# AppleHolic/pytorch_sound

Hardware: AMD Instinct MI355X
Metric: audio-sec/s STFT+mel+fwd/bwd (higher is better)
Workload: dtype bf16; 1 GPU; configs[1]: Conv1d separator (4 x ResBlock1, C=256, on 513-bin magnitude), 22.05 kHz, STFT 1024/256, 80 mel, batch 32 x 2 s per GPU, Adam, bf16 autocast; global_batch=32, parallelism=dp1, model_params=5520386

## Files before the change

### include/psnd.h

```cpp
#ifndef PSND_H
#define PSND_H

#include <stdint.h>
#include <stddef.h>

#ifdef __cplusplus
extern "C" {
#endif

#define PSND_OK 0
#define PSND_E_ARG (-1)
#define PSND_E_SHAPE (-2)
#define PSND_E_HIP (-3)
#define PSND_E_UNSUPPORTED (-4)

#define PSND_FRAMING_CENTER 0
#define PSND_FRAMING_HIFIGAN 1
#define PSND_FRAMING_NONE 2

int psnd_version(void);
const char *psnd_last_error(void);
#ifdef PSND_LAB
void psnd_env_refresh(void);
#endif
// ... 41 lines not shown
                  float eps, void *scratch, size_t scratch_bytes, float *out, void *stream);

#define PSND_LOG_NONE 0
#define PSND_LOG_E 1
#define PSND_LOG_10 2
size_t psnd_mel_plan_bytes(int M, int K);
int psnd_mel_plan_build(int M, int K, const float *mel_filter_host, void *plan_host);
int psnd_mel_fwd(const float *mag, int64_t N, int64_t F, int M, int K, const void *mel_plan,
                 int log_kind, float log_offset, float pre_clamp_min, float clamp_lo, float clamp_hi,
                 float *out, float *mel_lin, void *stream);
int psnd_mel_bwd(const float *gout, const float *mel_lin, int64_t N, int64_t F, int M, int K,
                 const void *mel_plan, int log_kind, float log_offset, float pre_clamp_min,
                 float clamp_lo, float clamp_hi, float *gmag, void *stream);

int psnd_logmel_fwd(const float *wav, int64_t N, int64_t T, int n_fft, int hop, int framing, const void *stft_plan,
                    float mag_eps, int M, const void *mel_plan, int log_kind, float log_offset, float pre_clamp_min,
                    float clamp_lo, float clamp_hi, float *out, void *stream);

int psnd_conv1d_cl(const void *A, const void *A2, const void *AM, float a2_slope, const void *W, const float *bias,
                   const void *res, const void *mask_src, int64_t N, int Lp, int L, int HP, int Ca, int Cb, int k,
                   int off0, int dstep, float act_slope, float mask_slope, void *out_raw, void *out_act,
                   void *a_eff_out, void *stream);
int psnd_conv1d_cl_wgrad_splits(int64_t N, int Lp, int Ca, int Cb, int k);
int psnd_conv1d_cl_pair_supported(int C, int k, int off1, int dstep1, int off2, int dstep2);
int psnd_conv1d_cl_pair(const void *A, const void *W1, const float *bias1, const void *M1, float m1_slope, float act1_slope,
                        void *mid_out, const void *W2, const float *bias2, const void *M2, float m2_slope, const void *res,
                        int64_t N, int Lp, int L, int HP, int C, int k, int off1, int dstep1, int off2, int dstep2,
                        float act2_slope, void *out_raw, void *out_act, void *stream);
typedef struct psnd_wgrad_desc {
    const void *g, *xa;
    float *gw_part, *gbias_part;
    int off0, dstep;
    int Ca, Cb, k, splits;
} psnd_wgrad_desc;
int psnd_conv1d_cl_wgrad_multi_splits(int64_t N, int Lp, int Ca, int Cb, int k, int n_convs);
int psnd_conv1d_cl_wgrad_multi(const psnd_wgrad_desc *d, int n, int64_t N, int Lp, void *stream);
typedef struct psnd_chain_pair {
    const void *W1;
    const float *bias1;
    float act1_slope;
    void *mid_out;
    const void *W2;
    const float *bias2;
    int off1, dstep1, off2, dstep2;
    float act2_slope;
    void *out_raw, *out_act;
// ... 18 lines not shown
int psnd_mel_l1_fwd_nfk(const float *mag_nfk, int64_t N, int64_t F, int M, int K, const void *mel_plan, int log_kind, float log_offset,
                        float pre_clamp_min, float clamp_lo, float clamp_hi, const float *ref, float *mel_lin, double *part, void *stream);
int psnd_mel_l1_bwd_nfk(const float *ref, const float *mel_lin, const float *g, float coef, int64_t N, int64_t F, int M, int K,
                        const void *mel_plan, int log_kind, float log_offset, float pre_clamp_min, float clamp_lo, float clamp_hi,
                        float *gmag_nfk, void *stream);
int64_t psnd_mask_head_l1_blocks(int64_t N, int64_t T, int Cp);
int psnd_mask_head_l1_fwd(const void *y, const float *mag, const float *ref, int64_t N, int C, int64_t T, int Lp, int HP, int Cp,
                          float *est, double *part, void *stream);
int psnd_mask_head_l1_bwd(const float *gest, const float *mag, const void *y, const float *est, const float *ref, const float *g,
                          float coef, int64_t N, int C, int64_t T, int Lp, int HP, int Cp, void *gy, void *stream);
int64_t psnd_mel_l1_blocks(int64_t N, int64_t F, int M);
int psnd_mel_l1_fwd(const float *mag, int64_t N, int64_t F, int M, int K, const void *mel_plan, int log_kind, float log_offset,
                    float pre_clamp_min, float clamp_lo, float clamp_hi, const float *ref, float *mel_lin, double *part, void *stream);
int psnd_mel_l1_bwd(const float *ref, const float *mel_lin, const float *g, float coef, int64_t N, int64_t F, int M, int K,
                    const void *mel_plan, int log_kind, float log_offset, float pre_clamp_min, float clamp_lo, float clamp_hi,
                    float *gmag, void *stream);
int psnd_nan_flag(const float *x, int64_t n, float *flag, void *stream);
int psnd_l1_loss_combine(const double *const *parts, const int64_t *nb, const double *scale, int terms, float *out, float *nan_flag, void *stream);
int psnd_conv_stats(int64_t *out4, int reset);
int psnd_conv_pair_stats(int64_t *out4, int reset);
int psnd_conv1d_cl_wgrad(const void *G1, const void *G2, const void *GM, float g2_slope, const void *xa, int64_t N,
                         int Lp, int Ca, int Cb, int k, int off0, int dstep, float *gw_part, float *gbias_part,
                         void *g_out, void *stream);
int psnd_conv1d_prep(const float *v, const float *g, const float *bias, int Cout, int Cin, int k, int Cb, int Ca,
                     void *wf, void *wb, float *bias_padded, void *stream);
int psnd_convtr1d_prep(const float *v, const float *g, const float *bias, int Cin, int Cout, int K, int stride, int Cr, int Cip,
                       void *wf, void *wb, float *bias_rep, void *stream);
int psnd_convtr1d_prep_multi(const void *descs_dev, int n, int total_blocks, void *stream);
int psnd_convtr1d_cl_fwd(const void *xa, const void *wf, const float *bias_rep, int64_t N, int Lp, int L, int HP, int Cip, int Cr,
                         int stride, int padding, int LpO, int HPO, float act_slope, void *out_raw, void *out_act, void *stream);
int psnd_convtr1d_cl_wgrad_splits(int64_t N, int Lp, int Cip, int Cr, int stride);
int psnd_convtr1d_cl_bwd(const void *g_raw, const void *g_act, const void *act, float act_slope, const void *wb, const void *xa,
                         int64_t N, int Lp, int L, int HP, int Cip, int Cr, int stride, int padding, int LpO, int HPO, void *gx,
                         void *g_eff, float *gw_part, void *stream);
int psnd_convtr1d_wnorm_bwd(const float *gw_part, int splits, const float *v, const float *g, int Cin, int Cout, int K, int stride,
                            int Cr, int Cip, float *gv, float *gg, void *stream);
int psnd_cl_mean_act_fwd(const void *a, const void *b, const void *c, const void *d, int count, float slope, void *out, int64_t n,
                         void *stream);
int psnd_cl_mean_act_bwd(const void *g, const void *y, int count, float slope, void *gin, int64_t n, void *stream);
int psnd_cl_sum2(const void *const *a, int na, void *out_a, const void *const *b, int nb, void *out_b, int64_t n, void *stream);
int psnd_cl_colsum_splits(int64_t rows, int C);
int psnd_cl_colsum(const void *g, int64_t rows, int C, int Lp, int lo, int hi, float *part, float *out, void *stream);
int psnd_conv1d_prep_multi(const void *descs_dev, int n, int total_blocks, int max_row, int which, void *stream);
#define PSND_WNORM_MAX 32
typedef struct psnd_wnorm_desc {
    const float *gw_part, *gbias_part;
// ... 154 lines not shown
```

### pytorch_sound_amd/_lib.py

```python
import ctypes
import os
import numpy as np

_HERE = os.path.dirname(os.path.abspath(__file__))
LIB_PATH = os.environ.get('PSND_LIB', os.path.join(_HERE, 'libpsnd_hip.so'))

PSND_OK = 0
FRAMING_CENTER = 0
FRAMING_HIFIGAN = 1
FRAMING_NONE = 2
LOG_NONE, LOG_E, LOG_10 = 0, 1, 2

_c = ctypes
_P = _c.c_void_p
_I64 = _c.c_int64
_INT = _c.c_int
_F = _c.c_float
_D = _c.c_double
_U32 = _c.c_uint32
_U64 = _c.c_uint64

SIGNATURES = {
    'psnd_version': (_INT, []),
    'psnd_last_error': (_c.c_char_p, []),
# ... 3 lines not shown
    'psnd_stream_wait_event': (_INT, [_P, _P]),
    'psnd_event_external_supported': (_INT, []),
    'psnd_frame_count': (_I64, [_I64, _INT, _INT, _INT]),
    'psnd_frame_sample_index': (_I64, [_I64, _INT, _I64, _INT, _INT, _INT]),
    'psnd_stft_plan_bytes': (_c.c_size_t, [_INT]),
    'psnd_stft_plan_build': (_INT, [_INT, _P, _P]),
    'psnd_stft_fwd': (_INT, [_P, _I64, _I64, _INT, _INT, _INT, _P, _F, _P, _P, _P, _P, _P]),
    'psnd_stft_mag_nfk': (_INT, [_P, _I64, _I64, _INT, _INT, _INT, _P, _F, _P, _P]),
    'psnd_stft_bwd': (_INT, [_P, _I64, _I64, _INT, _INT, _INT, _P, _F, _P, _P, _P, _P, _P]),
    'psnd_istft': (_INT, [_P, _P, _I64, _I64, _INT, _INT, _P, _F, _P, _P]),
    'psnd_stft_mr_plan_bytes': (_c.c_size_t, [_INT]),
    'psnd_stft_mr_plan_build': (_INT, [_INT, _P, _P]),
    'psnd_stft_mr_fwd': (_INT, [_P, _I64, _I64, _INT, _INT, _INT, _P, _c.c_size_t, _F, _P, _P, _P, _P, _P]),
    'psnd_stft_mr_bwd_scratch_bytes': (_c.c_size_t, [_I64, _I64, _INT, _INT, _INT]),
    'psnd_stft_mr_bwd': (_INT, [_P, _I64, _I64, _INT, _INT, _INT, _P, _c.c_size_t, _F, _P, _P, _P, _P, _c.c_size_t, _P, _P]),
    'psnd_istft_mr_scratch_bytes': (_c.c_size_t, [_I64, _I64, _INT]),
    'psnd_istft_mr': (_INT, [_P, _P, _I64, _I64, _INT, _INT, _P, _c.c_size_t, _F, _P, _c.c_size_t, _P, _P]),
    'psnd_mel_plan_bytes': (_c.c_size_t, [_INT, _INT]),
    'psnd_mel_plan_build': (_INT, [_INT, _INT, _P, _P]),
    'psnd_mel_fwd': (_INT, [_P, _I64, _I64, _INT, _INT, _P, _INT, _F, _F, _F, _F, _P, _P, _P]),
    'psnd_mel_bwd': (_INT, [_P, _P, _I64, _I64, _INT, _INT, _P, _INT, _F, _F, _F, _F, _P, _P]),
    'psnd_logmel_fwd': (_INT, [_P, _I64, _I64, _INT, _INT, _INT, _P, _F, _INT, _P, _INT, _F, _F, _F, _F, _P, _P]),
    'psnd_conv1d_cl': (_INT, [_P, _P, _P, _F, _P, _P, _P, _P, _I64, _INT, _INT, _INT, _INT, _INT, _INT, _INT, _INT, _F, _F, _P, _P, _P, _P]),
    'psnd_conv1d_cl_pair_supported': (_INT, [_INT, _INT, _INT, _INT, _INT, _INT]),
    'psnd_conv1d_cl_pair': (_INT, [_P, _P, _P, _P, _F, _F, _P, _P, _P, _P, _F, _P, _I64, _INT, _INT, _INT, _INT, _INT, _INT, _INT, _INT, _INT, _F, _P, _P, _P]),
    'psnd_conv1d_cl_wgrad': (_INT, [_P, _P, _P, _F, _P, _I64, _INT, _INT, _INT, _INT, _INT, _INT, _P, _P, _P, _P]),
    'psnd_conv1d_prep': (_INT, [_P, _P, _P, _INT, _INT, _INT, _INT, _INT, _P, _P, _P, _P]),
    'psnd_conv1d_wnorm_bwd': (_INT, [_P, _P, _INT, _P, _P, _INT, _INT, _INT, _INT, _INT, _P, _P, _P, _P]),
    'psnd_conv1d_cl_bwd': (_INT, [_P, _P, _P, _F, _P, _P, _I64, _INT, _INT, _INT, _INT, _INT, _INT, _INT, _INT, _P, _P, _P, _F, _P, _P, _P, _P]),
    'psnd_conv1d_cl_wgrad_multi_splits': (_INT, [_I64, _INT, _INT, _INT, _INT, _INT]),
    'psnd_conv1d_cl_wgrad_multi': (_INT, [_P, _INT, _I64, _INT, _P]),
    'psnd_nan_flag': (_INT, [_P, _I64, _P, _P]),
    'psnd_conv1d_cl_chain_rows': (_INT, [_INT, _INT, _INT, _P]),
    'psnd_conv1d_cl_chain_plan': (_INT, [_INT, _INT, _INT, _P, _I64, _P]),
    'psnd_conv1d_cl_chain': (_INT, [_P, _P, _P, _INT, _I64, _INT, _INT, _INT, _INT, _INT, _P]),
    'psnd_conv_chain_stats': (None, [_P]),
    'psnd_conv1d_cl_pair_bwd_supported': (_INT, [_INT, _INT, _INT, _INT, _INT, _INT]),
    'psnd_conv1d_cl_pair_bwd_splits': (_INT, [_I64, _INT, _INT, _INT]),
    'psnd_conv1d_cl_pair_bwd': (_INT, [_P, _P, _P, _F, _P, _P, _P, _F, _P, _I64, _INT, _INT, _INT, _INT, _INT, _INT, _INT, _INT, _INT, _P, _P, _P, _P,
                                       _P, _P, _INT, _INT, _P, _P, _P]),
    'psnd_conv1d_wnorm_bwd_multi': (_INT, [_P, _INT, _P]),
    'psnd_conv1d_prep_multi': (_INT, [_P, _INT, _INT, _INT, _INT, _P]),
    'psnd_conv1d_cl_wgrad_splits': (_INT, [_I64, _INT, _INT, _INT, _INT]),
    'psnd_mask_head_l1_blocks': (_I64, [_I64, _I64, _INT]),
    'psnd_masked_l1_blocks': (_I64, [_I64]),
    'psnd_masked_l1_fwd': (_INT, [_P, _P, _P, _I64, _INT, _I64, _P, _P, _P, _P]),
# ... 238 lines not shown
```

### pytorch_sound_amd/cl.py

```python
import ctypes
from collections import namedtuple
from pytorch_sound_amd import _switches as _sw
import weakref

import torch

from . import _lib
from ._lib import lib, check, ptr, stream_ptr

ALIGN_C = 32


def round_up(x, m):
    return (x + m - 1) // m * m


class CLShape:

    def __init__(self, N, L, HP):
        self.N, self.L, self.HP = int(N), int(L), int(HP)
        self.Lp = round_up(self.L + 2 * self.HP, 8)

    @property
    def R(self):
# ... 398 lines not shown

def branch_streams(dev, n):
    pool = _BRANCH_STREAMS.setdefault(dev.index, [])
    while len(pool) < n:
        pool.append(torch.cuda.Stream(device=dev))
    return pool[:n]


_WGRAD_STREAMS = {}


def _wgrad_streams(dev):
    if _sw.lab('PSND_CL_BWD_SPLIT', '0') != '1' or not _pair_enabled() or not AUTO_SECTIONS:
        return []
    n = int(_sw.lab('PSND_CL_WGRAD_STREAMS', '3'))
    pool = _WGRAD_STREAMS.setdefault(dev.index, [])
    while len(pool) < n:
        pool.append(torch.cuda.Stream(device=dev))
    return pool[:n]


def _pair_enabled():
    return _sw.lab('PSND_CL_PAIR', '1') != '0'


_Step = namedtuple('_Step', 'Cout Cin k Ca Cb dil pad slope has_res has_bias role')
_Conv = namedtuple('_Conv', 'inp wf bp res Ca Cb k off0 dil oslope raw act')
_Pair = namedtuple('_Pair', 'inp1 wf1 bp1 slope1 mid wf2 bp2 res C k off1 dstep1 off2 dstep2 oslope raw act')
_Chain = namedtuple('_Chain', 'inp1 res C k pairs')
_B = namedtuple('_B', 'G1 G2 am slope wb inp Ca Cb k pad dil gx g_out ep_mask ep_slope ep_res gw gbp S')
_W = namedtuple('_W', 'G1 G2 am slope inp Ca Cb k off0 dil gw gbp S')
_Side = namedtuple('_Side', 'w')
_PairB = namedtuple('_PairB', 'G wb2 m1 m1s g_h wb1 m2 m2s res C k off1 dstep1 off2 dstep2 gx flush_after')
_ChainB = namedtuple('_ChainB', 'pairs')
_PB = namedtuple('_PB', 'G wb2 m1 m1s g_h wb1 m2 m2s C k pad2 dil2 pad1 dil1 gx gw gbp lag')
_PBFlush = namedtuple('_PBFlush', 'lag')
_Lag = namedtuple('_Lag', 'g xa off0 dstep gw gbp C k')
_WBatch = namedtuple('_WBatch', 'conv G inp off0 dstep')


def _chain_takes(pairs):
    taps = [t for p in pairs for t in (p.off1, p.dstep1, p.off2, p.dstep2)]
    return lib().psnd_conv1d_cl_chain_rows(pairs[0].C, pairs[0].k, len(pairs), (ctypes.c_int * len(taps))(*taps)) >= 32


def _chain_pairs_bwd(plan, rows):
# ... 416 lines not shown
            last = i == n - 1
            inp, slope, has_res = src, (last_act_slope if last else 0.1), role in ('c2', 'r2')
            mk = lambda: torch.empty((shape.N, shape.Lp, Cb), dtype=torch.bfloat16, device=dev)
            if role == 'c1':
                raw, act, res, oslope = None, mk(), None, slope
                pending = act
            elif role == 'tail':
                raw, act, res, oslope = mk(), None, None, 1.0
                cur_x, cur_xa = raw, None
            else:
                raw, act, res, oslope = (mk() if (not last) or want_raw else None), mk(), (cur_x if has_res else None), slope
                cur_x, cur_xa = raw, act
            c1 = plan[-1] if plan else None
            if (role == 'c2' and _pair_enabled() and isinstance(c1, _Conv) and steps[-1].role == 'c1' and c1.Ca == Ca == Cb
                    and c1.k == k and lib().psnd_conv1d_cl_pair_supported(Ca, k, c1.off0, c1.dil, -pad, dil)):
                plan[-1] = _Pair(c1.inp, c1.wf, c1.bp, c1.oslope, c1.act, wf, bp, res, Ca, k, c1.off0, c1.dil, -pad, dil, oslope, raw, act)
            else:
                plan.append(_Conv(inp, wf, bp, res, Ca, Cb, k, -pad, dil, oslope, raw, act))
            steps.append(_Step(Cout, Cin, k, Ca, Cb, dil, pad, slope, has_res, b is not None, role))
            saved += [inp, act if act is not None else inp, wb, v32, g32]
        nsec, sides = _sections(dev, shape.N, shape.N * shape.Lp)
        Nh = shape.N // nsec
        plan = _chain_pairs(plan, Nh * shape.Lp)

        def run(h):
            st = stream_ptr(dev)
            q = lambda t: ptr(_sec(t, h, nsec))
            for e in plan:
                if isinstance(e, _Chain):
                    inp1, res0, C, k, pairs = e
                    arr = (_lib.ChainPair * len(pairs))()
                    for d, p in zip(arr, pairs):
                        d.W1, d.bias1, d.act1_slope, d.mid_out = p.wf1.data_ptr(), p.bp1.data_ptr(), float(p.slope1), q(p.mid)
                        d.W2, d.bias2, d.off1, d.dstep1, d.off2, d.dstep2 = p.wf2.data_ptr(), p.bp2.data_ptr(), p.off1, p.dstep1, p.off2, p.dstep2
                        d.act2_slope, d.out_raw, d.out_act = float(p.oslope), (q(p.raw) if p is pairs[-1] else None), q(p.act)
                    check(lib().psnd_conv1d_cl_chain(q(inp1), q(res0), ctypes.addressof(arr), len(pairs), Nh, shape.Lp, shape.L, shape.HP,
                                                     C, k, st), 'psnd_conv1d_cl_chain')
                    continue
                if isinstance(e, _Pair):
                    inp1, wf1, bp1, slope1, mid, wf2, bp2, res, C, k, off1, dstep1, off2, dstep2, oslope, raw, act = e
                    check(lib().psnd_conv1d_cl_pair(q(inp1), ptr(wf1), ptr(bp1), None, 1.0, float(slope1), q(mid), ptr(wf2), ptr(bp2),
                                                    None, 1.0, q(res), Nh, shape.Lp, shape.L, shape.HP, C, k, off1, dstep1, off2, dstep2,
                                                    float(oslope), q(raw), q(act), st), 'psnd_conv1d_cl_pair')
                    continue
                inp, wf, bp, res, Ca, Cb, k, off0, dil, oslope, raw, act = e
                check(lib().psnd_conv1d_cl(q(inp), None, None, 1.0, ptr(wf), ptr(bp), q(res), None,
                                           Nh, shape.Lp, shape.L, shape.HP, Ca, Cb, k, off0, dil, float(oslope), 1.0,
                                           q(raw), q(act), None, st), 'psnd_conv1d_cl')

        with torch.cuda.device(dev):
            _run_sections(dev, nsec, sides, run)
        ctx.steps, ctx.shape = steps, shape
        ctx.param_refs = params
        note_param_use(ctx, *params)
        ctx.save_for_backward(*saved)
        return cur_x, cur_xa

    @staticmethod
    def backward(ctx, g_raw, g_act):
        saved, steps, shape = ctx.saved_tensors, ctx.steps, ctx.shape
        dev = saved[0].device
        n = len(steps)
        if ctx.pack_owner is not None:
            ctx.pack_owner.write_backward_packs()
        g_raw = None if g_raw is None else g_raw.contiguous()
        g_act = None if g_act is None else g_act.contiguous()
        grads = [None] * (3 * n)
        descs, keep = [None] * n, []
# ... 8 lines not shown
                pv, pg, pb = prefs[3 * i:3 * i + 3]
                gv, gg = sink.dest(pv, pv.numel()), sink.dest(pg, pg.numel())
                gb = sink.dest(pb, Cb) if pb is not None else None
                early[i] = [(0, pv) if gv is not None else None, (1, pg) if gg is not None else None,
                            (2, pb) if gb is not None else None]
            gv = torch.empty_like(v32) if gv is None else gv.view_as(v32)
            gg = torch.empty_like(g32) if gg is None else gg.view_as(g32)
            gb = torch.empty(Cb, dtype=torch.float32, device=dev) if gb is None else gb
            return gv, gg, gb

        nsec, sides = _sections(dev, shape.N, shape.N * shape.Lp)
        wstreams = _wgrad_streams(dev) if shape.N * shape.Lp <= 8192 else []
        if wstreams:
            nsec, sides = 1, []
        Nh = shape.N // nsec
        plan = []
        skip = -1
        batch = (nsec == 1 and not wstreams and _pair_enabled() and _sw.lab('PSND_CL_BWD_BATCH', '1') == '1'
                 and shape.N * shape.Lp <= 8192)
        wbatch = []
        own_launch = []
        pair_bwd = nsec == 1 and not wstreams and not batch and _pair_enabled() and shape.N * shape.Lp <= 8192
        lag = None
        with torch.cuda.device(dev):
            g_comb = None
            res_pending = None
            def slabs(i, G1, G2, am, inp, S=None):
                s = steps[i]
                v32, g32 = saved[5 * i + 3], saved[5 * i + 4]
                if S is None:
                    S = lib().psnd_conv1d_cl_wgrad_splits(Nh, shape.Lp, s.Ca, s.Cb, s.k)
                gw = torch.empty((nsec * S, s.k, s.Cb, s.Ca), dtype=torch.float32, device=dev)
                gbp = torch.empty((nsec * S, s.Cb), dtype=torch.float32, device=dev)
                gv, gg, gb = grad_out(i, v32, g32, s.Cb)
                descs[i] = _lib.WnormDesc(gw.data_ptr(), gbp.data_ptr(), v32.data_ptr(), g32.data_ptr(), gv.data_ptr(), gg.data_ptr(),
                                          gb.data_ptr(), nsec * S, s.Cout, s.Cin, s.k, s.Cb, s.Ca)
                keep.extend([gw, gbp, G1, G2])
                grads[3 * i], grads[3 * i + 1] = gv, gg
                grads[3 * i + 2] = gb[:s.Cout] if s.has_bias else None
                return _W(G1, G2, am, s.slope, inp, s.Ca, s.Cb, s.k, -s.pad, s.dil, gw, gbp, S)

            for i in range(n - 1, -1, -1):
                if i == skip:
                    continue
                Cout, Cin, k, Ca, Cb, dil, pad, slope, has_res, has_bias, role = steps[i]
                inp, act, wb = saved[5 * i:5 * i + 3]
# ... 15 lines not shown
                        wl = slabs(i - 1, g_h, None, None, inp1, S2)
                        lag = _Lag(g_h, inp1, -p.pad, p.dil, wl.gw, wl.gbp, Ca, k)
                    else:
                        if batch:
                            wbatch += [_WBatch(i, G, inp, -pad, dil), _WBatch(i - 1, g_h, inp1, -p.pad, p.dil)]
                        else:
                            plan.append(_Side(slabs(i, G, None, None, inp)))
                        plan.append(_PairB(G, wb, inp, m1s, g_h, wb1, inp1, m2s, G, Ca, k, pad, -dil, p.pad, -p.dil, gx, len(wbatch)))
                        if not batch:
                            plan.append(_Side(slabs(i - 1, g_h, None, None, inp1)))
                    keep.extend([g_h, gx])
                    res_pending = G
                    g_comb = gx
                    skip = i - 1
                    continue
                if g_comb is None:
                    if g_raw is None and g_act is None:
                        raise _lib.PsndError('CL conv chain backward: no incoming gradient')
                    G1, G2 = g_raw, g_act
                    am = act if g_act is not None else None
                    need_gout = has_res and g_act is not None
                else:
                    G1, G2, am, need_gout = g_comb, None, None, False
                w = slabs(i, G1, G2, am, inp)
                g_out = torch.empty((shape.N, shape.Lp, Cb), dtype=torch.bfloat16, device=dev) if need_gout else None
                keep.append(g_out)
                g_here = g_out if need_gout else G1
                if i == 0 and not (ctx.needs_input_grad[0] or ctx.needs_input_grad[1]):
                    gx = None
                    plan.append(_Side(w) if wstreams else w)
                else:
                    gx = torch.empty((shape.N, shape.Lp, Ca), dtype=torch.bfloat16, device=dev)
                    if i == 0:
                        ep_mask, ep_res = None, None
                    elif role == 'c1':
                        ep_mask, ep_res = inp, res_pending
                    elif role == 'r2':
                        ep_mask, ep_res = inp, g_here
                    else:
                        ep_mask, ep_res = inp, None
                    plan.append(_B(G1, G2, am, slope, wb, inp, Ca, Cb, k, pad, dil, gx, g_out, ep_mask,
                                   float(p.slope if i > 0 else 1.0), ep_res, w.gw, w.gbp, w.S))
                own_launch.append((plan[-1], i))
                if role == 'c2':
                    res_pending = g_here
                if i > 0:
                    g_comb = gx
# ... 40 lines not shown
                        check(lib().psnd_conv1d_cl_pair_bwd(None, None, None, 1.0, None, None, None, 1.0, None, shape.N, shape.Lp, shape.L,
                                                            shape.HP, lg.C, lg.k, 0, 1, 0, 1, None, None, None, None, ptr(lg.g), ptr(lg.xa),
                                                            lg.off0, lg.dstep, ptr(lg.gw), ptr(lg.gbp), st), 'psnd_conv1d_cl_pair_bwd')
                        continue
                    if isinstance(e, _ChainB):
                        arr = (_lib.ChainPair * len(e.pairs))()
                        for d, p in zip(arr, e.pairs):
                            d.W1, d.bias1, d.act1_slope, d.mid_out = p.wb2.data_ptr(), None, 1.0, p.g_h.data_ptr()
                            d.W2, d.bias2, d.off1, d.dstep1, d.off2, d.dstep2 = p.wb1.data_ptr(), None, p.off1, p.dstep1, p.off2, p.dstep2
                            d.act2_slope, d.out_raw, d.out_act = 1.0, p.gx.data_ptr(), None
                            d.M1, d.M2, d.m1_slope, d.m2_slope = p.m1.data_ptr(), p.m2.data_ptr(), p.m1s, p.m2s
                        p0 = e.pairs[0]
                        check(lib().psnd_conv1d_cl_chain(ptr(p0.G), ptr(p0.G), ctypes.addressof(arr), len(e.pairs), shape.N, shape.Lp, shape.L,
                                                         shape.HP, p0.C, p0.k, st), 'psnd_conv1d_cl_chain')
                        continue
                    if isinstance(e, _PairB):
                        G, wb2, m1, m1s, g_h, wb1, m2, m2s, res, C, k, off1, dstep1, off2, dstep2, gx, _ = e
                        check(lib().psnd_conv1d_cl_pair(ptr(G), ptr(wb2), None, ptr(m1), m1s, 1.0, ptr(g_h), ptr(wb1), None, ptr(m2), m2s,
                                                        ptr(res), shape.N, shape.Lp, shape.L, shape.HP, C, k, off1, dstep1, off2, dstep2, 1.0,
                                                        ptr(gx), None, st), 'psnd_conv1d_cl_pair')
                        continue
                    if isinstance(e, _W):
                        G1, G2, am, slope, inp, Ca, Cb, k, off0, dil, gw, gbp, S = e
                        check(lib().psnd_conv1d_cl_wgrad(q(G1), q(G2), q(am), float(slope), q(inp), Nh, shape.Lp, Ca, Cb, k, off0, dil,
                                                         ptr(gw[h * S:(h + 1) * S]), ptr(gbp[h * S:(h + 1) * S]), None, st),
                              'psnd_conv1d_cl_wgrad')
                    else:
                        G1, G2, am, slope, wb, inp, Ca, Cb, k, pad, dil, gx, g_out, ep_mask, ep_slope, ep_res, gw, gbp, S = e
                        check(lib().psnd_conv1d_cl_bwd(q(G1), q(G2), q(am), float(slope), ptr(wb), q(inp), Nh, shape.Lp, shape.L,
                                                       shape.HP, Ca, Cb, k, pad, dil, q(gx), q(g_out), q(ep_mask), ep_slope, q(ep_res),
                                                       ptr(gw[h * S:(h + 1) * S]), ptr(gbp[h * S:(h + 1) * S]), st),
                              'psnd_conv1d_cl_bwd')

            st = stream_ptr(dev)
            handed = set()

            def wgrad_batch(part):
                for j0 in range(0, len(part), 32):
                    sub = part[j0:j0 + 32]
                    shp = [(steps[b.conv].Ca, steps[b.conv].Cb, steps[b.conv].k) for b in sub]
                    Ca, Cb, k = max(set(shp), key=shp.count)
                    cnt = max(shp.count((Ca, Cb, k)), len(wbatch) // 2) if len(part) < len(wbatch) else shp.count((Ca, Cb, k))
                    Sb = lib().psnd_conv1d_cl_wgrad_multi_splits(shape.N, shape.Lp, Ca, Cb, k, cnt)
                    arr = (_lib.WgradDesc * len(sub))()
                    for d, b in zip(arr, sub):
                        w = slabs(b.conv, b.G, None, None, b.inp, Sb)
# ... 119 lines not shown
```

### pytorch_sound_amd/csrc/psnd_conv.hip

```cpp
#include "psnd_common.h"
#include "psnd_conv_pair.h"
#include <stdlib.h>
#include <string.h>
#include <algorithm>
#include <atomic>

namespace {

typedef __attribute__((ext_vector_type(8))) short bf16x8;
typedef __attribute__((ext_vector_type(16))) float f32x16;
typedef unsigned short bf16_t;

__device__ __forceinline__ float bf2f(bf16_t v) { return __builtin_bit_cast(float, (unsigned)v << 16); }
__device__ __forceinline__ bf16_t f2bf(float f) {
    unsigned u = __builtin_bit_cast(unsigned, f);
    if ((u & 0x7fffffffu) > 0x7f800000u) return (bf16_t)((u >> 16) | 0x40);
    u += 0x7fffu + ((u >> 16) & 1u);
    return (bf16_t)(u >> 16);
}

typedef __bf16 hwbf16x2 __attribute__((ext_vector_type(2)));
typedef float f32x2_t __attribute__((ext_vector_type(2)));
__device__ __forceinline__ unsigned pack_bf16(float lo, float hi) {
    const f32x2_t v = {lo, hi};
// ... 1712 lines not shown
    const int wk = narrow_w ? 4 * WKT : pair_wk(k <= 3 ? 3 : (k <= 7 ? 7 : (k <= 11 ? 11 : 16)), 25);
    const int tx = (Cb + 63) / 64, ty = (Ca + 63) / 64 * ((k + wk - 1) / wk);
    int64_t target = 192;
    if (narrow_w) {
        target = 192;
        if (const char *e = PSND_ENV("PSND_WGRAD_BLOCKS_NARROW")) target = psnd_env_int(e, target, 1, 65535);
    }
    if (const char *e = PSND_ENV("PSND_WGRAD_BLOCKS")) target = psnd_env_int(e, target, 1, 65535);
    int64_t splits = target / ((int64_t)tx * ty);
    if (splits < 1) splits = 1;
    int64_t rps = (R + splits - 1) / splits;
    rps = (rps + 31) / 32 * 32;
    if (rps < 64) rps = 64;
    splits = (R + rps - 1) / rps;
    if (rps_out) *rps_out = rps;
    return (int)splits;
}

extern "C" int psnd_conv1d_cl_wgrad_splits(int64_t N, int Lp, int Ca, int Cb, int k) {
    if (N <= 0 || Lp <= 0 || Ca <= 0 || Cb <= 0 || k <= 0) return 0;
    return wgrad_splits(N * (int64_t)Lp, Ca, Cb, k, nullptr);
}

extern "C" int psnd_conv1d_cl_wgrad(const void *G1, const void *G2, const void *GM, float g2_slope, const void *xa, int64_t N,
                                    int Lp, int Ca, int Cb, int k, int off0, int dstep, float *gw_part, float *gbias_part,
                                    void *g_out, void *stream) {
    if ((!G1 && !G2) || (G2 && !GM) || !xa || !gw_part) PSND_FAIL(PSND_E_ARG, "conv1d_cl_wgrad: null pointer");
    if (Ca % 8 != 0 || Cb % 8 != 0 || k < 1 || k > 16 || N < 0) PSND_FAIL(PSND_E_SHAPE, "conv1d_cl_wgrad: Ca=%d Cb=%d k=%d", Ca, Cb, k);
    if ((k < WKT ? k - 1 : WKT - 1) * (dstep < 0 ? -dstep : dstep) > WXR - 32)
        PSND_FAIL(PSND_E_UNSUPPORTED, "conv1d_cl_wgrad: dilation %d: a tap group spans more than %d rows", dstep, WXR - 32);
    if (N == 0) return PSND_OK;
    if ((size_t)N * Lp * (Ca > Cb ? Ca : Cb) * 2 >= ((size_t)1 << 32)) PSND_FAIL(PSND_E_SHAPE, "conv1d_cl_wgrad: operand larger than 4 GB");
    WgradParams p;
    wgrad_params_plain(p);
    p.G1 = static_cast<const bf16_t *>(G1), p.G2 = static_cast<const bf16_t *>(G2), p.GM = static_cast<const bf16_t *>(GM);
    p.xa = static_cast<const bf16_t *>(xa), p.gw = gw_part, p.gbias = gbias_part, p.g_out = static_cast<bf16_t *>(g_out);
    p.R = N * (int64_t)Lp, p.Ca = Ca, p.Cb = Cb, p.k = k, p.off0 = off0, p.dstep = dstep, p.g2_slope = g2_slope;
    const int tx = (Cb + 63) / 64, ty = (Ca + 63) / 64;
    int64_t rps;
    const int splits = wgrad_splits(p.R, Ca, Cb, k, &rps);
    p.rows_per_split = (int)rps;
#ifdef PSND_TRACE
    {
        const char *tp = PSND_ENV("PSND_TRACE_PTR");
        p.trace = tp ? reinterpret_cast<long long *>(strtoull(tp, nullptr, 0)) : nullptr;
    }
#endif
    hipLaunchKernelGGL(conv_wgrad_kernel, dim3(tx, ty, (unsigned)(splits * ((k + WKT - 1) / WKT))), dim3(256), kWgradLdsBytes,
                       static_cast<hipStream_t>(stream), p);
    PSND_CHECK_LAUNCH("conv1d_cl_wgrad");
    return PSND_OK;
}

static int wgrad_multi_splits(int64_t R, int Ca, int Cb, int k, int n, int64_t *rps_out) {
    const int tiles = ((Ca + 63) / 64) * ((Cb + 63) / 64) * ((k + WKT - 1) / WKT);
    int64_t target = 768;
    if (const char *e = PSND_ENV("PSND_WGRAD_MULTI_BLOCKS")) target = psnd_env_int(e, target, 1, 65535);
    int64_t splits = target / ((int64_t)tiles * (n > 0 ? n : 1));
    if (splits < 1) splits = 1;
    int64_t rps = (R + splits - 1) / splits;
    rps = (rps + 31) / 32 * 32;
    if (rps < 64) rps = 64;
    splits = (R + rps - 1) / rps;
    if (rps_out) *rps_out = rps;
    return (int)splits;
}

extern "C" int psnd_conv1d_cl_wgrad_multi_splits(int64_t N, int Lp, int Ca, int Cb, int k, int n_convs) {
    if (N <= 0 || Lp <= 0 || Ca <= 0 || Cb <= 0 || k <= 0 || n_convs <= 0) return 0;
    return wgrad_multi_splits(N * (int64_t)Lp, Ca, Cb, k, n_convs, nullptr);
}

extern "C" int psnd_conv1d_cl_wgrad_multi(const psnd_wgrad_desc *d, int n, int64_t N, int Lp, void *stream) {
    if (!d || n < 0) PSND_FAIL(PSND_E_ARG, "conv1d_cl_wgrad_multi: null pointer");
// ... 781 lines not shown
```

### pytorch_sound_amd/csrc/psnd_core.hip

```cpp
#include "psnd_common.h"

static thread_local char g_err[512] = "";

void psnd_set_error(const char *fmt, ...) {
    va_list ap;
    va_start(ap, fmt);
    vsnprintf(g_err, sizeof(g_err), fmt, ap);
    va_end(ap);
}

extern "C" int psnd_version(void) { return 141; }

extern "C" const char *psnd_last_error(void) { return g_err; }

#ifdef PSND_LAB
std::atomic<int> g_psnd_env_gen{0};
extern "C" void psnd_env_refresh(void) { g_psnd_env_gen.fetch_add(1, std::memory_order_acq_rel); }
#endif

static inline int64_t pad_of(int n_fft, int hop, int framing) {
    if (framing == PSND_FRAMING_NONE) return 0;
    return framing == PSND_FRAMING_CENTER ? n_fft / 2 : (n_fft - hop) / 2;
}

extern "C" int64_t psnd_frame_count(int64_t T, int n_fft, int hop, int framing) {
    if (T <= 0 || n_fft <= 0 || hop <= 0) return 0;
    const int64_t L = T + 2 * pad_of(n_fft, hop, framing);
    if (L < n_fft) return 0;
    return (L - n_fft) / hop + 1;
}

extern "C" int64_t psnd_frame_sample_index(int64_t f, int m, int64_t T, int n_fft, int hop, int framing) {
    int64_t i = f * hop - pad_of(n_fft, hop, framing) + m;
    if (i < 0) i = -i;
// ... 106 lines not shown
```

Baseline: 107,000 audio-s/s.

## Add wide-input conv1d kernel and higher-split wgrad for first layer

Adds a dedicated forward conv kernel for the case where many input channels (e.g. 513-bin magnitude padded) map to 256 output channels with k=3. Each 512-thread block stages an input row tile in LDS and streams weights from registers via MFMA 32x32x16. It also gives the first layer's weight-gradient, when no input grad is needed, its own split count aimed at about 504 blocks, to fill the GPU better. The cost is more code paths and extra partial-sum buffers, and the fixed tile choice may suit some shapes poorly.

New measurement: 106,700 audio-s/s. No clear change (-0.3%).

```diff
diff --git a/include/psnd.h b/include/psnd.h
--- a/include/psnd.h
+++ b/include/psnd.h
@@ -87,6 +87,9 @@
                    int off0, int dstep, float act_slope, float mask_slope, void *out_raw, void *out_act,
                    void *a_eff_out, void *stream);
 int psnd_conv1d_cl_wgrad_splits(int64_t N, int Lp, int Ca, int Cb, int k);
+int psnd_conv1d_cl_wide_supported(int Ca, int Cb, int k, int off0, int dstep);
+int psnd_conv1d_cl_wide(const void *A, const void *W, const float *bias, int64_t N, int Lp, int L, int HP, int Ca, int Cb, int k,
+                        int off0, int dstep, float act_slope, void *out_raw, void *out_act, void *stream);
 int psnd_conv1d_cl_pair_supported(int C, int k, int off1, int dstep1, int off2, int dstep2);
 int psnd_conv1d_cl_pair(const void *A, const void *W1, const float *bias1, const void *M1, float m1_slope, float act1_slope,
                         void *mid_out, const void *W2, const float *bias2, const void *M2, float m2_slope, const void *res,
@@ -151,6 +154,10 @@
 int psnd_conv1d_cl_wgrad(const void *G1, const void *G2, const void *GM, float g2_slope, const void *xa, int64_t N,
                          int Lp, int Ca, int Cb, int k, int off0, int dstep, float *gw_part, float *gbias_part,
                          void *g_out, void *stream);
+int psnd_conv1d_cl_wgrad_splits_alone(int64_t N, int Lp, int Ca, int Cb, int k);
+int psnd_conv1d_cl_wgrad_ex(const void *G1, const void *G2, const void *GM, float g2_slope, const void *xa, int64_t N,
+                            int Lp, int Ca, int Cb, int k, int off0, int dstep, int splits, float *gw_part, float *gbias_part,
+                            void *g_out, void *stream);
 int psnd_conv1d_prep(const float *v, const float *g, const float *bias, int Cout, int Cin, int k, int Cb, int Ca,
                      void *wf, void *wb, float *bias_padded, void *stream);
 int psnd_convtr1d_prep(const float *v, const float *g, const float *bias, int Cin, int Cout, int K, int stride, int Cr, int Cip,
diff --git a/pytorch_sound_amd/_lib.py b/pytorch_sound_amd/_lib.py
--- a/pytorch_sound_amd/_lib.py
+++ b/pytorch_sound_amd/_lib.py
@@ -49,6 +49,10 @@
     'psnd_mel_bwd': (_INT, [_P, _P, _I64, _I64, _INT, _INT, _P, _INT, _F, _F, _F, _F, _P, _P]),
     'psnd_logmel_fwd': (_INT, [_P, _I64, _I64, _INT, _INT, _INT, _P, _F, _INT, _P, _INT, _F, _F, _F, _F, _P, _P]),
     'psnd_conv1d_cl': (_INT, [_P, _P, _P, _F, _P, _P, _P, _P, _I64, _INT, _INT, _INT, _INT, _INT, _INT, _INT, _INT, _F, _F, _P, _P, _P, _P]),
+    'psnd_conv1d_cl_wide_supported': (_INT, [_INT, _INT, _INT, _INT, _INT]),
+    'psnd_conv1d_cl_wide': (_INT, [_P, _P, _P, _I64, _INT, _INT, _INT, _INT, _INT, _INT, _INT, _INT, _F, _P, _P, _P]),
+    'psnd_conv1d_cl_wgrad_splits_alone': (_INT, [_I64, _INT, _INT, _INT, _INT]),
+    'psnd_conv1d_cl_wgrad_ex': (_INT, [_P, _P, _P, _F, _P, _I64, _INT, _INT, _INT, _INT, _INT, _INT, _INT, _P, _P, _P, _P]),
     'psnd_conv1d_cl_pair_supported': (_INT, [_INT, _INT, _INT, _INT, _INT, _INT]),
     'psnd_conv1d_cl_pair': (_INT, [_P, _P, _P, _P, _F, _F, _P, _P, _P, _P, _F, _P, _I64, _INT, _INT, _INT, _INT, _INT, _INT, _INT, _INT, _INT, _F, _P, _P, _P]),
     'psnd_conv1d_cl_wgrad': (_INT, [_P, _P, _P, _F, _P, _I64, _INT, _INT, _INT, _INT, _INT, _INT, _P, _P, _P, _P]),
diff --git a/pytorch_sound_amd/cl.py b/pytorch_sound_amd/cl.py
--- a/pytorch_sound_amd/cl.py
+++ b/pytorch_sound_amd/cl.py
@@ -444,6 +444,10 @@
 
 def _pair_enabled():
     return _sw.lab('PSND_CL_PAIR', '1') != '0'
+
+
+def _wide_enabled():
+    return _sw.lab('PSND_CL_WIDE', '1') != '0'
 
 
 _Step = namedtuple('_Step', 'Cout Cin k Ca Cb dil pad slope has_res has_bias role')
@@ -906,6 +910,7 @@
         nsec, sides = _sections(dev, shape.N, shape.N * shape.Lp)
         Nh = shape.N // nsec
         plan = _chain_pairs(plan, Nh * shape.Lp)
+        wide = _wide_enabled()
 
         def run(h):
             st = stream_ptr(dev)
@@ -928,6 +933,11 @@
                                                     float(oslope), q(raw), q(act), st), 'psnd_conv1d_cl_pair')
                     continue
                 inp, wf, bp, res, Ca, Cb, k, off0, dil, oslope, raw, act = e
+                if (res is None and Ca > Cb and wide and Nh * shape.Lp * Ca * 2 < 2 ** 31
+                        and lib().psnd_conv1d_cl_wide_supported(Ca, Cb, k, off0, dil)):
+                    check(lib().psnd_conv1d_cl_wide(q(inp), ptr(wf), ptr(bp), Nh, shape.Lp, shape.L, shape.HP, Ca, Cb, k, off0, dil,
+                                                    float(oslope), q(raw), q(act), st), 'psnd_conv1d_cl_wide')
+                    continue
                 check(lib().psnd_conv1d_cl(q(inp), None, None, 1.0, ptr(wf), ptr(bp), q(res), None,
                                            Nh, shape.Lp, shape.L, shape.HP, Ca, Cb, k, off0, dil, float(oslope), 1.0,
                                            q(raw), q(act), None, st), 'psnd_conv1d_cl')
@@ -982,6 +992,7 @@
         own_launch = []
         pair_bwd = nsec == 1 and not wstreams and not batch and _pair_enabled() and shape.N * shape.Lp <= 8192
         lag = None
+        alone_w = None
         with torch.cuda.device(dev):
             g_comb = None
             res_pending = None
@@ -1043,7 +1054,10 @@
                     need_gout = has_res and g_act is not None
                 else:
                     G1, G2, am, need_gout = g_comb, None, None, False
-                w = slabs(i, G1, G2, am, inp)
+                alone = i == 0 and not (ctx.needs_input_grad[0] or ctx.needs_input_grad[1]) and not wstreams and not sides
+                w = slabs(i, G1, G2, am, inp, lib().psnd_conv1d_cl_wgrad_splits_alone(Nh, shape.Lp, Ca, Cb, k) if alone else None)
+                if alone:
+                    alone_w = w
                 g_out = torch.empty((shape.N, shape.Lp, Cb), dtype=torch.bfloat16, device=dev) if need_gout else None
                 keep.append(g_out)
                 g_here = g_out if need_gout else G1
@@ -1130,6 +1144,11 @@
                         continue
                     if isinstance(e, _W):
                         G1, G2, am, slope, inp, Ca, Cb, k, off0, dil, gw, gbp, S = e
+                        if e is alone_w:
+                            check(lib().psnd_conv1d_cl_wgrad_ex(q(G1), q(G2), q(am), float(slope), q(inp), Nh, shape.Lp, Ca, Cb, k, off0, dil, S,
+                                                                ptr(gw[h * S:(h + 1) * S]), ptr(gbp[h * S:(h + 1) * S]), None, st),
+                                  'psnd_conv1d_cl_wgrad_ex')
+                            continue
                         check(lib().psnd_conv1d_cl_wgrad(q(G1), q(G2), q(am), float(slope), q(inp), Nh, shape.Lp, Ca, Cb, k, off0, dil,
                                                          ptr(gw[h * S:(h + 1) * S]), ptr(gbp[h * S:(h + 1) * S]), None, st),
                               'psnd_conv1d_cl_wgrad')
diff --git a/pytorch_sound_amd/csrc/psnd_conv.hip b/pytorch_sound_amd/csrc/psnd_conv.hip
--- a/pytorch_sound_amd/csrc/psnd_conv.hip
+++ b/pytorch_sound_amd/csrc/psnd_conv.hip
@@ -1758,9 +1758,37 @@
     return wgrad_splits(N * (int64_t)Lp, Ca, Cb, k, nullptr);
 }
 
-extern "C" int psnd_conv1d_cl_wgrad(const void *G1, const void *G2, const void *GM, float g2_slope, const void *xa, int64_t N,
-                                    int Lp, int Ca, int Cb, int k, int off0, int dstep, float *gw_part, float *gbias_part,
-                                    void *g_out, void *stream) {
+static int64_t wgrad_rows_per_split(int64_t R, int splits) {
+    if (splits < 1 || R < 1) return 0;
+    int64_t rps = ((R + splits - 1) / splits + 31) / 32 * 32;
+    if (rps < 64) rps = 64;
+    if ((R + rps - 1) / rps != splits) rps = (R + splits - 1) / splits;
+    return (R + rps - 1) / rps == splits ? rps : 0;
+}
+
+static int wgrad_splits_alone(int64_t R, int Ca, int Cb, int k) {
+    const int base = wgrad_splits(R, Ca, Cb, k, nullptr);
+    if (Ca <= 32 && Cb <= 32) return base;
+    const int wk = pair_wk(k <= 3 ? 3 : (k <= 7 ? 7 : (k <= 11 ? 11 : 16)), 25);
+    const int tiles = (Cb + 63) / 64 * ((Ca + 63) / 64) * ((k + wk - 1) / wk);
+    int64_t target = 504;
+    if (const char *e = PSND_ENV("PSND_WGRAD_BLOCKS_ALONE")) target = psnd_env_int(e, (int)target, 1, 65535);
+    int64_t splits = target / tiles;
+    if (splits > 16) splits = 16;
+    if (splits < base) return base;
+    int64_t rps = ((R + splits - 1) / splits + 31) / 32 * 32;
+    if (rps < 64) rps = 64;
+    return (int)((R + rps - 1) / rps);
+}
+
+extern "C" int psnd_conv1d_cl_wgrad_splits_alone(int64_t N, int Lp, int Ca, int Cb, int k) {
+    if (N <= 0 || Lp <= 0 || Ca <= 0 || Cb <= 0 || k <= 0) return 0;
+    return wgrad_splits_alone(N * (int64_t)Lp, Ca, Cb, k);
+}
+
+extern "C" int psnd_conv1d_cl_wgrad_ex(const void *G1, const void *G2, const void *GM, float g2_slope, const void *xa, int64_t N,
+                                       int Lp, int Ca, int Cb, int k, int off0, int dstep, int splits, float *gw_part, float *gbias_part,
+                                       void *g_out, void *stream) {
     if ((!G1 && !G2) || (G2 && !GM) || !xa || !gw_part) PSND_FAIL(PSND_E_ARG, "conv1d_cl_wgrad: null pointer");
     if (Ca % 8 != 0 || Cb % 8 != 0 || k < 1 || k > 16 || N < 0) PSND_FAIL(PSND_E_SHAPE, "conv1d_cl_wgrad: Ca=%d Cb=%d k=%d", Ca, Cb, k);
     if ((k < WKT ? k - 1 : WKT - 1) * (dstep < 0 ? -dstep : dstep) > WXR - 32)
@@ -1773,8 +1801,9 @@
     p.xa = static_cast<const bf16_t *>(xa), p.gw = gw_part, p.gbias = gbias_part, p.g_out = static_cast<bf16_t *>(g_out);
     p.R = N * (int64_t)Lp, p.Ca = Ca, p.Cb = Cb, p.k = k, p.off0 = off0, p.dstep = dstep, p.g2_slope = g2_slope;
     const int tx = (Cb + 63) / 64, ty = (Ca + 63) / 64;
-    int64_t rps;
-    const int splits = wgrad_splits(p.R, Ca, Cb, k, &rps);
+    const int64_t rps = wgrad_rows_per_split(p.R, splits);
+    if (rps == 0 || splits * (int64_t)((k + WKT - 1) / WKT) > 65535)
+        PSND_FAIL(PSND_E_SHAPE, "conv1d_cl_wgrad: %d row ranges over %lld rows", splits, (long long)p.R);
     p.rows_per_split = (int)rps;
 #ifdef PSND_TRACE
     {
@@ -1786,6 +1815,13 @@
                        static_cast<hipStream_t>(stream), p);
     PSND_CHECK_LAUNCH("conv1d_cl_wgrad");
     return PSND_OK;
+}
+
+extern "C" int psnd_conv1d_cl_wgrad(const void *G1, const void *G2, const void *GM, float g2_slope, const void *xa, int64_t N,
+                                    int Lp, int Ca, int Cb, int k, int off0, int dstep, float *gw_part, float *gbias_part,
+                                    void *g_out, void *stream) {
+    const int splits = (N > 0 && Lp > 0 && Ca > 0 && Cb > 0 && k >= 1 && k <= 16) ? wgrad_splits(N * (int64_t)Lp, Ca, Cb, k, nullptr) : 1;
+    return psnd_conv1d_cl_wgrad_ex(G1, G2, GM, g2_slope, xa, N, Lp, Ca, Cb, k, off0, dstep, splits, gw_part, gbias_part, g_out, stream);
 }
 
 static int wgrad_multi_splits(int64_t R, int Ca, int Cb, int k, int n, int64_t *rps_out) {
diff --git a/pytorch_sound_amd/csrc/psnd_conv_wide.hip b/pytorch_sound_amd/csrc/psnd_conv_wide.hip
--- /dev/null
+++ b/pytorch_sound_amd/csrc/psnd_conv_wide.hip
@@ -0,0 +1,218 @@
+#include "psnd_conv_pair.h"
+
+namespace {
+using namespace pairk;
+
+constexpr int WIDE_CB = 256;
+constexpr int WIDE_OS = WIDE_CB + 8;
+constexpr int WIDE_HDR = 1024 + 64;
+
+struct WideParams {
+    const bf16_t *A;
+    const bf16_t *W;
+    const float *bias;
+    bf16_t *out_raw, *out_act;
+    long long R;
+    int Lp, L, HP, Ca, CaP, off0, dstep, hm;
+    float act_slope;
+    long long *trace;
+};
+#ifdef PSND_TRACE
+#define WIDE_STAMP(i_)                                                                                                                    \
+    do {                                                                                                                                  \
+        if (p.trace && (threadIdx.x & 63) == 0) p.trace[((size_t)blockIdx.x * 8 + (threadIdx.x >> 6)) * 8 + (i_)] = __builtin_amdgcn_s_memtime(); \
+    } while (0)
+#else
+#define WIDE_STAMP(i_)
+#endif
+
+template <int MR>
+__global__ __launch_bounds__(512, 1) void conv_wide_kernel(WideParams p) {
+    constexpr int NT = 512, RU = 12, AR = 3, MROWS = 32 * MR, MB = MR, OS = WIDE_OS, NB = 10;
+    extern __shared__ __attribute__((aligned(16))) unsigned char smem_w[];
+    float *s_bias = reinterpret_cast<float *>(smem_w);
+    unsigned char *s_in = smem_w + 1024;
+    bf16_t *sX = reinterpret_cast<bf16_t *>(smem_w + WIDE_HDR);
+    const int RS = p.CaP + 8, BR = MROWS + 2 * p.hm, PCS = p.CaP >> 3, KSTEPS = p.Ca >> 4;
+    bf16_t *sOr = sX + BR * RS, *sOa = sOr + MROWS * OS;
+    const int tid = threadIdx.x, wave = tid >> 6, lane = tid & 63, li = lane & 31, kg = lane >> 5;
+    const long long r0 = (long long)blockIdx.x * MROWS;
+    const unsigned a_bytes = (unsigned)((size_t)p.R * p.Ca * sizeof(bf16_t)), o_bytes = (unsigned)((size_t)p.R * WIDE_CB * sizeof(bf16_t));
+    const unsigned w_bytes = (unsigned)(3u * WIDE_CB * (unsigned)p.Ca * sizeof(bf16_t));
+    const __amdgpu_buffer_rsrc_t rA = make_uniform_rsrc(p.A, (int)a_bytes), rW = make_uniform_rsrc(p.W, (int)w_bytes);
+    WIDE_STAMP(0);
+
+    uint4 rb[RU];
+    const unsigned fwave = (unsigned)wave * (unsigned)KSTEPS * 1024u + (unsigned)lane * 16u;
+    const unsigned ftap = (unsigned)(WIDE_CB / 32) * (unsigned)KSTEPS * 1024u;
+    auto fetch_b = [&](auto slotc, int it) __attribute__((always_inline)) {
+        constexpr int slot = decltype(slotc)::value, tap = (slot % 6) / 2, ksl = 2 * (slot / 6) + slot % 2;
+        const int ks = 4 * it + ksl;
+        rb[slot] = __builtin_bit_cast(uint4, __builtin_amdgcn_raw_buffer_load_b128(rW, (int)(ks < KSTEPS ? fwave : OOB),
+                                                                                    (int)((unsigned)tap * ftap + (unsigned)ks * 1024u), 0));
+    };
+    static_for<0, RU>([&](auto uc) __attribute__((always_inline)) { fetch_b(uc, 0); });
+    {
+        const int q512 = NT / PCS, r512 = NT - q512 * PCS;
+        int row = tid / PCS, pc = tid - row * PCS;
+        for (int base = 0; base < BR * PCS; base += NB * NT) {
+            uint4 ra[NB];
+            int lo[NB];
+#pragma unroll
+            for (int u = 0; u < NB; ++u) {
+                const long long r = r0 - p.hm + row;
+                const bool ok = row < BR && r >= 0 && r < p.R && 8 * pc < p.Ca;
+                ra[u] = ld16(rA, ok ? (unsigned)(((size_t)r * p.Ca + 8 * pc) * sizeof(bf16_t)) : OOB);
+                lo[u] = row < BR ? row * RS + 8 * pc : -1;
+                row += q512, pc += r512;
+                if (pc >= PCS) pc -= PCS, ++row;
+            }
+#pragma unroll
+            for (int u = 0; u < NB; ++u)
+                if (lo[u] >= 0) *reinterpret_cast<uint4 *>(sX + lo[u]) = ra[u];
+        }
+    }
+    if (tid < WIDE_CB) s_bias[tid] = p.bias ? p.bias[tid] : 0.f;
+    if (tid < MROWS) {
+        const long long r = r0 + tid;
+        const int l = (int)(r % p.Lp);
+        s_in[tid] = (r < p.R && l >= p.HP && l < p.HP + p.L) ? 1 : 0;
+    }
+    __syncthreads();
+    WIDE_STAMP(1);
+
+    f32x16 acc[MB];
+#pragma unroll
+    for (int m = 0; m < MB; ++m)
+#pragma unroll
+        for (int i = 0; i < 16; ++i) acc[m][i] = 0.f;
+    const bf16_t *ab[3][MB];
+#pragma unroll
+    for (int t = 0; t < 3; ++t)
+#pragma unroll
+        for (int m = 0; m < MB; ++m) ab[t][m] = sX + (m * 32 + li + p.hm + p.off0 + t * p.dstep) * RS + 8 * kg;
+    auto afrag = [&](auto uc, bf16x8 (&x)[MB]) __attribute__((always_inline)) {
+        constexpr int u = decltype(uc)::value, tap = (u % 6) / 2, ch = 32 * (u / 6) + 16 * (u % 2);
+#pragma unroll
+        for (int m = 0; m < MB; ++m) x[m] = *reinterpret_cast<const bf16x8 *>(ab[tap][m] + ch);
+    };
+    bf16x8 xr[AR][MB];
+    static_for<0, AR - 1>([&](auto uc) __attribute__((always_inline)) { afrag(uc, xr[decltype(uc)::value]); });
+    const int turns = (p.CaP >> 6);
+#pragma unroll 1
+    for (int it = 0; it < turns; ++it) {
+        static_for<0, RU>([&](auto uc) __attribute__((always_inline)) {
+            constexpr int u = decltype(uc)::value;
+            afrag(std::integral_constant<int, u + AR - 1>{}, xr[(u + AR - 1) % AR]);
+            const bf16x8 b = __builtin_bit_cast(bf16x8, rb[u]);
+#pragma unroll
+            for (int m = 0; m < MB; ++m) acc[m] = __builtin_amdgcn_mfma_f32_32x32x16_bf16(b, xr[u % AR][m], acc[m], 0, 0, 0);
+            fetch_b(uc, it + 1);
+            __builtin_amdgcn_sched_group_barrier(0x100, MB, 0);
+            __builtin_amdgcn_sched_group_barrier(0x008, MB, 0);
+            __builtin_amdgcn_sched_group_barrier(0x020, 1, 0);
+            __builtin_amdgcn_sched_barrier(0);
+        });
+#pragma unroll
+        for (int t = 0; t < 3; ++t)
+#pragma unroll
+            for (int m = 0; m < MB; ++m) ab[t][m] += 64;
+    }
+    WIDE_STAMP(2);
+
+    const int cb = wave * 32 + 4 * kg, eo = li * OS + cb;
+    const float sl = p.act_slope;
+    const bool want_raw = p.out_raw != nullptr, want_act = p.out_act != nullptr;
+    float4 bb[4];
+#pragma unroll
+    for (int g = 0; g < 4; ++g) bb[g] = *reinterpret_cast<const float4 *>(&s_bias[cb + 8 * g]);
+#pragma unroll
+    for (int m = 0; m < MB; ++m) {
+        const unsigned rmask = s_in[m * 32 + li] ? 0xffffffffu : 0u;
+#pragma unroll
+        for (int g = 0; g < 4; ++g) {
+            const float v0 = acc[m][4 * g] + bb[g].x, v1 = acc[m][4 * g + 1] + bb[g].y;
+            const float v2 = acc[m][4 * g + 2] + bb[g].z, v3 = acc[m][4 * g + 3] + bb[g].w;
+            if (want_raw)
+                *reinterpret_cast<uint2 *>(sOr + eo + m * 32 * OS + 8 * g) = make_uint2(pack_bf16(v0, v1) & rmask, pack_bf16(v2, v3) & rmask);
+            if (want_act)
+                *reinterpret_cast<uint2 *>(sOa + eo + m * 32 * OS + 8 * g) =
+                    make_uint2(pack_bf16(v0 > 0.f ? v0 : v0 * sl, v1 > 0.f ? v1 : v1 * sl) & rmask,
+                               pack_bf16(v2 > 0.f ? v2 : v2 * sl, v3 > 0.f ? v3 : v3 * sl) & rmask);
+        }
+    }
+    __syncthreads();
+    WIDE_STAMP(3);
+    auto copy_out = [&](const bf16_t *src, bf16_t *dst) __attribute__((always_inline)) {
+        const __amdgpu_buffer_rsrc_t rO = make_uniform_rsrc(dst, (int)o_bytes);
+#pragma unroll
+        for (int u = 0; u < MROWS * (WIDE_CB / 8) / NT; ++u) {
+            const int idx = tid + NT * u, i = idx >> 5, pc = idx & 31;
+            const long long r = r0 + i;
+            const uint4 v = *reinterpret_cast<const uint4 *>(src + i * OS + 8 * pc);
+            __builtin_amdgcn_raw_buffer_store_b128(__builtin_bit_cast(__attribute__((ext_vector_type(4))) unsigned, v), rO,
+                                                   (int)(r < p.R ? (unsigned)(((size_t)r * WIDE_CB + 8 * pc) * sizeof(bf16_t)) : OOB), 0, 0);
+        }
+    };
+    if (want_raw) copy_out(sOr, p.out_raw);
+    if (want_act) copy_out(sOa, p.out_act);
+    WIDE_STAMP(4);
+}
+
+int wide_mr() {
+    int mr = 1;
+    if (const char *e = PSND_ENV("PSND_CL_WIDE_MR")) {
+        const int f = atoi(e);
+        if (f == 1 || f == 2) mr = f;
+    }
+    return mr;
+}
+int wide_cap(int Ca) { return (Ca + 63) / 64 * 64; }
+size_t wide_lds(int Ca, int hm, int mr) {
+    return (size_t)WIDE_HDR + ((size_t)(32 * mr + 2 * hm) * (wide_cap(Ca) + 8) + (size_t)2 * 32 * mr * WIDE_OS) * sizeof(bf16_t);
+}
+}
+
+extern "C" int psnd_conv1d_cl_wide_supported(int Ca, int Cb, int k, int off0, int dstep) {
+    if (Cb != WIDE_CB || k != 3 || Ca < 32 || Ca % 32 != 0) return 0;
+    const int hm = reach3(off0, dstep);
+    if (hm > HMAXP) return 0;
+    return wide_lds(Ca, hm, wide_mr()) <= 160 * 1024 ? 1 : 0;
+}
+
+extern "C" int psnd_conv1d_cl_wide(const void *A, const void *W, const float *bias, int64_t N, int Lp, int L, int HP, int Ca, int Cb, int k,
+                                   int off0, int dstep, float act_slope, void *out_raw, void *out_act, void *stream) {
+    if (!A || !W || (!out_raw && !out_act)) PSND_FAIL(PSND_E_ARG, "conv1d_cl_wide: null pointer");
+    if (N < 0 || L <= 0 || HP < 0 || Lp < L + 2 * HP) PSND_FAIL(PSND_E_SHAPE, "conv1d_cl_wide: N=%lld Lp=%d L=%d HP=%d", (long long)N, Lp, L, HP);
+    if (!psnd_conv1d_cl_wide_supported(Ca, Cb, k, off0, dstep))
+        PSND_FAIL(PSND_E_UNSUPPORTED, "conv1d_cl_wide: Ca=%d Cb=%d k=%d taps %d%+d: only Cb = 256, k = 3, Ca a multiple of 32, reach <= %d, tile within 160 KB",
+                  Ca, Cb, k, off0, dstep, HMAXP);
+    const int hm = reach3(off0, dstep);
+    if (hm > HP) PSND_FAIL(PSND_E_UNSUPPORTED, "conv1d_cl_wide: tap reach %d exceeds the halo HP=%d", hm, HP);
+    if (N == 0) return PSND_OK;
+    if ((size_t)N * Lp * (Ca > Cb ? Ca : Cb) * 2 >= ((size_t)1 << 31)) PSND_FAIL(PSND_E_SHAPE, "conv1d_cl_wide: operand larger than 2 GB");
+    WideParams p;
+    p.A = static_cast<const bf16_t *>(A), p.W = static_cast<const bf16_t *>(W), p.bias = bias;
+    p.out_raw = static_cast<bf16_t *>(out_raw), p.out_act = static_cast<bf16_t *>(out_act);
+    p.R = N * (int64_t)Lp, p.Lp = Lp, p.L = L, p.HP = HP, p.Ca = Ca, p.CaP = wide_cap(Ca), p.off0 = off0, p.dstep = dstep, p.hm = hm;
+    p.act_slope = act_slope;
+    p.trace = nullptr;
+#ifdef PSND_TRACE
+    {
+        const char *tp = PSND_ENV("PSND_TRACE_PTR");
+        p.trace = tp ? reinterpret_cast<long long *>(strtoull(tp, nullptr, 0)) : nullptr;
+    }
+#endif
+    const int mr = wide_mr();
+    const size_t lds = wide_lds(Ca, hm, mr);
+    const int64_t tiles = (p.R + 32 * mr - 1) / (32 * mr);
+    hipStream_t st = static_cast<hipStream_t>(stream);
+    auto launch = [&](auto kern) {
+        (void)hipFuncSetAttribute(reinterpret_cast<const void *>(kern), hipFuncAttributeMaxDynamicSharedMemorySize, 160 * 1024);
+        hipLaunchKernelGGL(kern, dim3((unsigned)tiles), dim3(512), lds, st, p);
+    };
+    if (mr == 2) launch(conv_wide_kernel<2>);
+    else launch(conv_wide_kernel<1>);
+    PSND_CHECK_LAUNCH("conv1d_cl_wide");
+    return PSND_OK;
+}
diff --git a/pytorch_sound_amd/csrc/psnd_core.hip b/pytorch_sound_amd/csrc/psnd_core.hip
--- a/pytorch_sound_amd/csrc/psnd_core.hip
+++ b/pytorch_sound_amd/csrc/psnd_core.hip
@@ -9,7 +9,7 @@
     va_end(ap);
 }
 
-extern "C" int psnd_version(void) { return 141; }
+extern "C" int psnd_version(void) { return 142; }
 
 extern "C" const char *psnd_last_error(void) { return g_err; }
 
```
